# kaleo996/F5E-TTS

Measured on AMD Instinct MI355X. Metric: mel_frames_per_sec, higher is better.
Workload: dtype bf16; 1 GPU; C2: F5TTS_v1_Base random-init, batch 1 per GPU, N_ref=188 N=469 frames, euler NFE=32, CFG=2.0 (cond+uncond batched), sway=-1.0, hipGraph ODE loop, HIP log-mel front-end + Vocos decode on GPU; parallelism=replica x1 (utterance sharding, no collective on the data path)

## Files before the change

f5e-tts_amd/csrc/gemm_bf16.hip:

```cpp
#include <cstdlib>
#include <type_traits>

#include "f5e_common.h"
#include "gemm_bf16_args.h"

namespace {

using namespace f5e_gemm;

template <int N>
__device__ __forceinline__ void wait_vm_lgkm0() {
  asm volatile("s_waitcnt vmcnt(%0) lgkmcnt(0)" ::"n"(N) : "memory");
}

template <int LPT, int EXTRA>
__device__ __forceinline__ void wait_stages(int nst) {
  constexpr auto C = [](int v) constexpr { return v > 63 ? 63 : v; };
  switch (nst) {
    case 0: wait_vm_lgkm0<C(EXTRA)>(); break;
    case 1: wait_vm_lgkm0<C(LPT + EXTRA)>(); break;
    case 2: wait_vm_lgkm0<C(2 * LPT + EXTRA)>(); break;
    case 3: wait_vm_lgkm0<C(3 * LPT + EXTRA)>(); break;
    case 4: wait_vm_lgkm0<C(4 * LPT + EXTRA)>(); break;
    case 5: wait_vm_lgkm0<C(5 * LPT + EXTRA)>(); break;
    default: wait_vm_lgkm0<C(6 * LPT + EXTRA)>(); break;
  }
}

template <int BM, int BN, int EPI, int NSTAGE, int DBG = 0, int WGM = 2, int WGN = 2, int FUSE = 0, int NLOAD = 0, int DSTEP = 1, int DBUF = 1>
__global__ __launch_bounds__(64 * (WGM * WGN + NLOAD)) void gemm_bf16_kernel(GemmArgs a) {
  constexpr int BK = 64;
  constexpr int CPR = BK / 8;
  constexpr int ROWB = BK * 2;
  auto swz = [](int row) { return (row >> 1) & 7; };
  constexpr int NCW = WGM * WGN;
  constexpr int NC = 64 * NCW;
  constexpr int NT = NLOAD ? 64 * NLOAD : NC;
  constexpr int A_BYTES = BM * BK * 2;
  constexpr int W_BYTES = BN * BK * 2;
  constexpr int STAGE = A_BYTES + W_BYTES;
  constexpr int WM = BM / WGM, WN = BN / WGN;
  constexpr int TM = WM / 16, TN = WN / 16;
  extern __shared__ __attribute__((aligned(16))) char smem[];

  const int lane = threadIdx.x & 63;
  const int wave = __builtin_amdgcn_readfirstlane(threadIdx.x >> 6);
  const int tid = (int)threadIdx.x;
  const bool is_loader = NLOAD > 0 && wave >= NCW;
  const int stid = NLOAD ? tid - NC : tid;
  const int swave = NLOAD ? wave - NCW : wave;
  unsigned long long* trc = nullptr;
  if constexpr (DBG >= 3) {
    trc = a.trace + (size_t)blockIdx.x * 48;
    if (tid == 0) { trc[0] = __builtin_amdgcn_s_memrealtime(); trc[1] = __builtin_amdgcn_s_memtime(); }
  }

  if (FUSE == 1)
    asm volatile("" ::"s"(a.ln_stats), "s"(a.ln_c), "s"(a.ln_d), "s"(a.ln_parts), "s"(a.cd_stride), "s"(a.cd_rows),
                 "s"(a.cd_eval_stride), "s"(a.eval_ptr));
  if (EPI == EPI_GATE_RES)
    asm volatile("" ::"s"(a.resid), "s"(a.gate), "s"(a.seq_len), "s"(a.eval_ptr), "s"(a.ldr), "s"(a.gate_stride),
                 "s"(a.gate_rows), "s"(a.eval_stride), "s"(a.bias));
  if (FUSE == 2) asm volatile("" ::"s"(a.next_scale), "s"(a.xs_out), "s"(a.stats_out), "s"(a.ld_xs), "s"(a.row_mean));
  if (EPI == EPI_QKV_ROPE) asm volatile("" ::"s"(a.q), "s"(a.k), "s"(a.vt), "s"(a.cos_sin), "s"(a.n_pad), "s"(a.heads), "s"(a.rope_heads));

  if ((int)blockIdx.x >= a.n_main) {
    if (NLOAD > 0 && a.pf_per_wg) f5e_prefetch_run_packed(a.pf, (int)blockIdx.x - a.n_main, tid, 64 * (NCW + NLOAD), a.pf_per_wg, smem);
    else if (tid < 256) f5e_prefetch_run(a.pf, (int)blockIdx.x - a.n_main, tid, smem);
    return;
  }
  int bid = blockIdx.x;
  {
    const int nblk = a.n_main;
    const int q8 = nblk >> 3, r8 = nblk & 7;
    const int xcd = bid & 7, idx = bid >> 3;
    bid = (xcd < r8 ? xcd * (q8 + 1) : r8 * (q8 + 1) + (xcd - r8) * q8) + idx;
  }
  int tile_m, tile_n;
  if (a.m_major > 0) {
    tile_m = div_magic(bid, a.tiles_n, a.tile_magic);
    tile_n = bid - tile_m * a.tiles_n;
  } else {
    const int sh = -a.m_major, per = a.tiles_m << sh;
    const int g = div_magic(bid, per, a.tile_magic);
    const int r = bid - g * per;
    tile_m = r >> sh;
    tile_n = (g << sh) + (r & ((1 << sh) - 1));
  }
  const int m0 = tile_m * BM, n0 = tile_n * BN;

  constexpr int A_IT = BM * CPR / NT;
  constexpr int W_IT = BN * CPR / NT;
  static_assert(A_IT >= 1 && W_IT >= 1 && A_IT * NT == BM * CPR && W_IT * NT == BN * CPR, "tile / thread-count mismatch");
  unsigned a_off[A_IT], w_off[W_IT];
#pragma unroll
  for (int j = 0; j < A_IT; ++j) {
    const int i = (stid & (NT - 1)) + NT * j;
    const int row = i / CPR, c = (i % CPR) ^ swz(row);
    a_off[j] = (unsigned)(min(m0 + row, a.M - 1) - m0) * (unsigned)(a.lda * 2) + (unsigned)c * 16u;
  }
#pragma unroll
  for (int j = 0; j < W_IT; ++j) {
    const int i = (stid & (NT - 1)) + NT * j;
    const int row = i / CPR, c = (i % CPR) ^ swz(row);
    w_off[j] = (unsigned)(min(n0 + row, a.N - 1) - n0) * (unsigned)(a.ldw * 2) + (unsigned)c * 16u;
  }
  const char* const a_base = (const char*)(a.A + (size_t)m0 * a.lda);
  const char* const w_base = (const char*)(a.W + (size_t)n0 * a.ldw);
  const int KT = a.K / BK;
  char* const ring = smem;
  auto stage = [&](int buf, int kt) {
    char* base = ring + buf * STAGE;
    const char* ak = a_base + (size_t)kt * (BK * 2);
    const char* wk = w_base + (size_t)kt * (BK * 2);
#pragma unroll
    for (int j = 0; j < A_IT; ++j) glds16_s(ak, a_off[j], base + (swave * 64 + NT * j) * 16);
#pragma unroll
    for (int j = 0; j < W_IT; ++j) glds16_s(wk, w_off[j], base + A_BYTES + (swave * 64 + NT * j) * 16);
  };

  const int wm0 = (wave / WGN) * WM, wn0 = (wave % WGN) * WN;
  const int fr = lane & 15, fq = lane >> 4;

  f32x4 acc[TN][TM];
#pragma unroll
  for (int i = 0; i < TN; ++i)
#pragma unroll
    for (int j = 0; j < TM; ++j) acc[i][j] = f32x4{0.f, 0.f, 0.f, 0.f};

  constexpr int LPT = A_IT + W_IT;
  static_assert(NSTAGE >= 2 && NSTAGE <= 8 && (DSTEP > 1 || (NSTAGE - 2) * LPT <= 63), "vmcnt is a 6-bit counter");
  static_assert((NT & (NT - 1)) == 0, "staging thread count must be a power of two");
  static_assert(DSTEP == 1 || (NLOAD > 0 && DSTEP == 2 && NSTAGE >= 3 * DSTEP), "DSTEP: role split, ring of >= 3 steps");
  constexpr int NPRO = NSTAGE - DSTEP;
  static_assert((NSTAGE - 2 * DSTEP) * LPT <= 63, "vmcnt is a 6-bit counter");
  if (NLOAD == 0 || is_loader) {
#pragma unroll
    for (int s = 0; s < NPRO; ++s)
      if (s < KT) stage(s, s);
  }
  if constexpr (NLOAD > 0) {
    if (is_loader) {
      int nbuf_l = NPRO % NSTAGE;
      if constexpr (DBG >= 3) { if (stid == 0) trc[47] = __builtin_amdgcn_s_memtime(); }
      for (int kt = 0; kt < KT; kt += DSTEP) {
        const int rem = KT - DSTEP - kt;
        wait_stages<LPT, 0>(rem < NSTAGE - 2 * DSTEP ? (rem < 0 ? 0 : rem) : NSTAGE - 2 * DSTEP);
        __builtin_amdgcn_s_barrier();
#pragma unroll
        for (int d = 0; d < DSTEP; ++d) {
          if (kt + NPRO + d < KT) stage(nbuf_l, kt + NPRO + d);
          nbuf_l = (nbuf_l + 1 == NSTAGE) ? 0 : nbuf_l + 1;
        }
      }
      if (FUSE == 1) __syncthreads();
      if (FUSE == 2) __builtin_amdgcn_s_barrier();
      return;
    }
  }
  asm volatile("" ::: "memory");
  if constexpr (DBG >= 3) { if (tid == 0) trc[46] = __builtin_amdgcn_s_memtime(); }
  constexpr bool PREF = (TM * TN <= 4);
  static_assert(FUSE != 2 || (PREF && WM == 32 && WN == 32 && BN == 64 && (BM == 64 || (BM == 128 && NLOAD > 0))),
                "fused AdaLN producer: 64 (or, role split, 128) x 64 tiles of 32 x 32 wave sub-tiles");
  static_assert(FUSE != 1 || (WN == 32 && (BN == 64 || NLOAD > 0) && ((BM == 64 && WM == 32) || (BM == 128 && WM == 64 && NLOAD > 0))),
                "fused AdaLN consumer: 64-row tiles of 32 x 32 wave sub-tiles, or (role split) 128-row tiles of 64 x 32 ones");
  static_assert(DBUF == 1 || (NLOAD > 0 && DSTEP == 1), "single fragment set: role split, one tile per hand-over");
  constexpr int NSTATT = BM * 4;
  static_assert(FUSE != 1 || NSTATT <= NC, "fused consumer: 4 statistics threads per row");
  static_assert(FUSE != 2 || EPI == EPI_GATE_RES, "the AdaLN producer is the gate+residual epilogue");
  constexpr int NPC = NLOAD ? 0 : (FUSE == 1 ? 2 * TN + 4 : (FUSE == 2 ? 3 * TM * TN : ((PREF && EPI == EPI_GATE_RES) ? 2 * TM * TN : 0)));
  static_assert((NSTAGE - 2) * LPT + NPC <= 63, "vmcnt is a 6-bit counter");
  constexpr bool COLG = NLOAD > 0;
  f32x4 pf_bias[PREF ? TN : 1], pf_gate[PREF ? TN : 1][PREF ? (COLG ? 1 : TM) : 1], pf_x[PREF ? TN : 1][PREF ? TM : 1];
  f32x4 pf_c[FUSE == 1 ? TN : 1], pf_d[FUSE == 1 ? TN : 1];
  f32x4 pf_ns[FUSE == 2 ? TN : 1][FUSE == 2 ? (COLG ? 1 : TM) : 1];
  f32x2 pf_st[FUSE == 1 ? 4 : 1];
  bool pf_live[PREF ? TM : 1];
  int pf_len[PREF ? TM : 1];
  float pf_rm[FUSE == 2 ? TM : 1];
  auto ldv4 = [](const float* ptr) -> f32x4 { return *(const f32x4*)ptr; };
  auto fetch_epilogue_operands = [&]() {
    if (PREF) {
      if (EPI == EPI_GATE_RES) {
        const size_t eoff = a.eval_ptr ? (size_t)load_uniform_i32(a.eval_ptr) * a.eval_stride : 0;
#pragma unroll
        for (int j = 0; j < TM; ++j) {
          const int m = m0 + wm0 + j * 16 + fr, mc = min(m, a.M - 1);
          const int seq = div_magic(mc, a.rows_per_seq, a.rps_magic);
#pragma unroll
          for (int i = 0; i < TN; ++i) {
            const int nc = min(n0 + wn0 + i * 16 + fq * 4, a.N - 4);
            const size_t goff = eoff + ((COLG || a.gate_rows == 1) ? 0 : (size_t)(seq % a.gate_rows) * a.gate_stride) + nc;
            if (!COLG || j == 0) pf_gate[i][COLG ? 0 : j] = ldv4(a.gate + goff);
            pf_x[i][j] = ldv4(a.resid + (size_t)mc * a.ldr + nc);
            if (FUSE == 2 && (!COLG || j == 0)) pf_ns[i][COLG ? 0 : j] = ldv4(a.next_scale + goff);
          }
        }
      }
    }
    if (FUSE == 1) {
      const size_t eoff = a.eval_ptr ? (size_t)load_uniform_i32(a.eval_ptr) * a.cd_eval_stride : 0;
      const float* cbase = a.ln_c + eoff;
      const float* dbase = a.ln_d + eoff;
#pragma unroll
      for (int i = 0; i < TN; ++i) {
        const unsigned nc = (unsigned)min(n0 + wn0 + i * 16 + fq * 4, a.N - 4);
        pf_c[i] = ldv4(cbase + nc);
        pf_d[i] = ldv4(dbase + nc);
      }
      const int pp = a.ln_parts >> 2;
      const float* sbase = a.ln_stats + (size_t)m0 * a.ln_parts * 2;
      const unsigned rel_max = (unsigned)((a.M - m0) * a.ln_parts - 1);
#pragma unroll
      for (int u = 0; u < 4; ++u) {
        const unsigned rel = min((unsigned)((tid & (NSTATT - 1)) * pp + min(u, pp - 1)), rel_max);
        if (NC == NSTATT || tid < NSTATT) pf_st[u] = *(const f32x2*)(sbase + rel * 2u);
      }
    }
    if (PREF) {
#pragma unroll
      for (int i = 0; i < TN; ++i) {
        const int n = n0 + wn0 + i * 16 + fq * 4;
        pf_bias[i] = (a.bias && n < a.N) ? *(const f32x4*)(a.bias + n) : f32x4{0.f, 0.f, 0.f, 0.f};
      }
      if (EPI == EPI_GATE_RES) {
#pragma unroll
        for (int j = 0; j < TM; ++j) {
          const int mc = min(m0 + wm0 + j * 16 + fr, a.M - 1);
          pf_len[j] = a.seq_len ? a.seq_len[div_magic(mc, a.rows_per_seq, a.rps_magic)] : a.rows_per_seq;
          if (FUSE == 2) pf_rm[j] = a.row_mean[mc];
        }
      }
    }
  };
  if (NLOAD == 0) fetch_epilogue_operands();

  int buf = 0, nbuf = NSTAGE - 1;
  if constexpr (DBG >= 3) { if (tid == 0) trc[2] = __builtin_amdgcn_s_memtime(); }
  if constexpr (NLOAD > 0) {
    bf16x8 xs2[DBUF + 1][BK / 32][TM], ws2[DBUF + 1][BK / 32][TN];
    auto reads = [&](auto pc, int b) {
      constexpr int P = decltype(pc)::value;
      const char* As = ring + b * STAGE;
      const char* Ws = As + A_BYTES;
#pragma unroll
      for (int kk = 0; kk < BK / 32; ++kk) {
        const int c = kk * 4 + fq;
#pragma unroll
        for (int j = 0; j < TM; ++j) {
          const int row = wm0 + j * 16 + fr;
          xs2[P][kk][j] = *(const bf16x8*)(As + row * ROWB + ((c ^ swz(row)) << 4));
        }
#pragma unroll
        for (int i = 0; i < TN; ++i) {
          const int row = wn0 + i * 16 + fr;
          ws2[P][kk][i] = *(const bf16x8*)(Ws + row * ROWB + ((c ^ swz(row)) << 4));
        }
      }
    };
    auto mfmas = [&](auto pc) {
      constexpr int P = decltype(pc)::value;
#pragma unroll
      for (int kk = 0; kk < BK / 32; ++kk)
#pragma unroll
        for (int i = 0; i < TN; ++i)
#pragma unroll
          for (int j = 0; j < TM; ++j)
            acc[i][j] = __builtin_amdgcn_mfma_f32_16x16x32_bf16(ws2[P][kk][i], xs2[P][kk][j], acc[i][j], 0, 0, 0);
    };
    auto body = [&](auto pc, int kt) {
      constexpr int P = decltype(pc)::value;
      if (DSTEP == 1 || P == 0) __builtin_amdgcn_s_barrier();
      if constexpr (DBG >= 3) { if (tid == 0 && kt < 36) trc[4 + kt] = __builtin_amdgcn_s_memtime(); }
      reads(pc, buf);
      if (kt > 0) mfmas(std::integral_constant<int, 1 - P>{});
      if (DSTEP == 1 || P == 1) asm volatile("s_waitcnt lgkmcnt(0)" ::: "memory");
      buf = (buf + 1 == NSTAGE) ? 0 : buf + 1;
    };
    if constexpr (DBUF == 0) {
      auto reads_half = [&](int kk, int b) {
        if constexpr (DBG == 5) return;
        const char* As = ring + b * STAGE;
        const char* Ws = As + A_BYTES;
        const int c = kk * 4 + fq;
#pragma unroll
        for (int j = 0; j < TM; ++j) {
          const int row = wm0 + j * 16 + fr;
          xs2[0][kk][j] = *(const bf16x8*)(As + row * ROWB + ((c ^ swz(row)) << 4));
        }
#pragma unroll
        for (int i = 0; i < TN; ++i) {
          const int row = wn0 + i * 16 + fr;
          ws2[0][kk][i] = *(const bf16x8*)(Ws + row * ROWB + ((c ^ swz(row)) << 4));
        }
      };
      auto mfmas_half = [&](int kk) {
        if constexpr (DBG == 4 || DBG == 5) return;
#pragma unroll
        for (int i = 0; i < TN; ++i)
#pragma unroll
          for (int j = 0; j < TM; ++j)
            acc[i][j] = __builtin_amdgcn_mfma_f32_16x16x32_bf16(ws2[0][kk][i], xs2[0][kk][j], acc[i][j], 0, 0, 0);
      };
      static_assert(BK == 64, "half-tile pipelining: two 32-k halves per K-tile");
      for (int kt = 0; kt < KT; ++kt) {
        __builtin_amdgcn_s_barrier();
        if constexpr (DBG >= 3) { if (tid == 0 && kt < 36) trc[4 + kt] = __builtin_amdgcn_s_memtime(); }
        reads_half(0, buf);
        if (kt > 0) mfmas_half(1);
        if (kt == 0) fetch_epilogue_operands();
        asm volatile("s_waitcnt lgkmcnt(0)" ::: "memory");
        reads_half(1, buf);
        mfmas_half(0);
        asm volatile("s_waitcnt lgkmcnt(0)" ::: "memory");
        buf = (buf + 1 == NSTAGE) ? 0 : buf + 1;
      }
      mfmas_half(1);
    } else {
      for (int kt = 0; kt < KT; kt += 2) {
        body(std::integral_constant<int, 0>{}, kt);
        if (kt == 0) fetch_epilogue_operands();
        if (kt + 1 < KT) body(std::integral_constant<int, 1>{}, kt + 1);
      }
      if ((KT - 1) & 1) mfmas(std::integral_constant<int, 1>{});
      else mfmas(std::integral_constant<int, 0>{});
    }
  } else
  for (int kt = 0; kt < KT; ++kt) {
    const int rem = KT - 1 - kt;
    const int nst = rem < NSTAGE - 2 ? rem : NSTAGE - 2;
    if (NPC > 0 && kt <= NSTAGE - 2) wait_stages<LPT, NPC>(nst);
    else wait_stages<LPT, 0>(nst);
    __builtin_amdgcn_s_barrier();
    if constexpr (DBG >= 3) { if (tid == 0 && kt < 36) trc[4 + kt] = __builtin_amdgcn_s_memtime(); }
    const bool more = kt + NSTAGE - 1 < KT;
    const char* As = ring + buf * STAGE;
    const char* Ws = As + A_BYTES;
    bf16x8 xf[BK / 32][TM], wf[BK / 32][TN];
#pragma unroll
    for (int kk = 0; kk < BK / 32; ++kk) {
      const int c = kk * 4 + fq;
#pragma unroll
      for (int j = 0; j < TM; ++j) {
        const int row = wm0 + j * 16 + fr;
        xf[kk][j] = *(const bf16x8*)(As + row * ROWB + ((c ^ swz(row)) << 4));
      }
#pragma unroll
      for (int i = 0; i < TN; ++i) {
        const int row = wn0 + i * 16 + fr;
        wf[kk][i] = *(const bf16x8*)(Ws + row * ROWB + ((c ^ swz(row)) << 4));
      }
    }
    if (more) stage(nbuf, kt + NSTAGE - 1);
#pragma unroll
    for (int kk = 0; kk < BK / 32; ++kk)
#pragma unroll
      for (int i = 0; i < TN; ++i)
#pragma unroll
        for (int j = 0; j < TM; ++j)
          acc[i][j] = __builtin_amdgcn_mfma_f32_16x16x32_bf16(wf[kk][i], xf[kk][j], acc[i][j], 0, 0, 0);
    buf = (buf + 1 == NSTAGE) ? 0 : buf + 1;
    nbuf = (nbuf + 1 == NSTAGE) ? 0 : nbuf + 1;
  }

  if constexpr (DBG >= 3) { if (tid == 0) trc[3] = __builtin_amdgcn_s_memtime(); }
  float* fuse_lds = (float*)(smem + NSTAGE * STAGE);
  if (FUSE == 1) {
    const int sq = tid & 3, pp = a.ln_parts >> 2;
    float sm = 0.f;
#pragma unroll
    for (int u = 0; u < 4; ++u)
      if (u < pp) sm += pf_st[u][0];
    sm = add_xor2(add_xor1(sm));
    const float mean = sm / (float)a.ln_parts;
    const float cols = (float)(a.K / a.ln_parts);
    float m2 = 0.f;
#pragma unroll
    for (int u = 0; u < 4; ++u)
      if (u < pp) {
        const float dm = pf_st[u][0] - mean;
        m2 += pf_st[u][1] + cols * dm * dm;
      }
    m2 = add_xor2(add_xor1(m2));
    if (sq == 0 && (NC == NSTATT || tid < NSTATT)) {
      fuse_lds[(tid >> 2) * 2] = mean;
      fuse_lds[(tid >> 2) * 2 + 1] = rsqrtf(m2 / (float)a.K + a.ln_eps);
      if (tile_n == 0 && m0 + (tid >> 2) < a.M) a.row_mean[m0 + (tid >> 2)] += mean;
    }
    __syncthreads();
    if constexpr (DBG >= 3) { if (tid == 0) trc[42] = __builtin_amdgcn_s_memtime(); }
  }
  f32x4 xn[FUSE == 2 ? TN : 1][FUSE == 2 ? TM : 1];
  if (PREF && EPI == EPI_GATE_RES) {
#pragma unroll
    for (int j = 0; j < TM; ++j) {
      const int m = m0 + wm0 + j * 16 + fr;
      pf_live[j] = (m < a.M) && (m - div_magic(m, a.rows_per_seq, a.rps_magic) * a.rows_per_seq < pf_len[j]);
    }
  }

  int qkv_which = 0, qkv_head = 0, qkv_d0 = 0;
  bf16* qkv_base = nullptr;
  size_t qkv_seq_stride = 0;
  if (EPI == EPI_QKV_ROPE) {
    static_assert(EPI != EPI_QKV_ROPE || WN <= 64, "a wave's columns must stay inside one 64-wide head");
    const int inner = a.heads * 64, hb = n0 + wn0;
    qkv_which = hb / inner;
    qkv_head = (hb - qkv_which * inner) >> 6;
    qkv_d0 = hb & 63;
    qkv_seq_stride = (size_t)a.heads * a.n_pad * 64;
    qkv_base = (qkv_which == 0 ? a.q : (qkv_which == 1 ? a.k : a.vt)) + (size_t)qkv_head * a.n_pad * 64;
  }

#pragma unroll
  for (int j = 0; j < TM; ++j) {
    const int m = m0 + wm0 + j * 16 + fr;
    if (FUSE == 2) {
#pragma unroll
      for (int i = 0; i < TN; ++i) xn[i][j] = pf_x[i][j];
    }
    if (m >= a.M) continue;
    float ln_mean = 0.f, ln_rstd = 1.f;
    if (FUSE == 1) {
      ln_mean = fuse_lds[(wm0 + j * 16 + fr) * 2];
      ln_rstd = fuse_lds[(wm0 + j * 16 + fr) * 2 + 1];
    }
    int seq = 0, pos = m;
    if (EPI == EPI_GATE_RES || EPI == EPI_QKV_ROPE) {
      seq = div_magic(m, a.rows_per_seq, a.rps_magic);
      pos = m - seq * a.rows_per_seq;
    }
    float qk_rn = 1.0f;
    const float* qk_w = nullptr;
    if constexpr (EPI == EPI_QKV_ROPE && WN == 64) {
      const int which_w = (n0 + wn0) / (a.heads * 64);
      if (a.qn_w && which_w < 2) {
        float ss = 0.f;
#pragma unroll
        for (int i = 0; i < TN; ++i) {
          f32x4 t = acc[i][j];
          if (a.bias) t += *(const f32x4*)(a.bias + n0 + wn0 + i * 16 + fq * 4);
          ss += (t[0] * t[0] + t[1] * t[1]) + (t[2] * t[2] + t[3] * t[3]);
        }
        ss = add_xor32(add_xor16(ss));
        qk_rn = rsqrtf(ss * (1.0f / 64.0f) + a.qk_eps);
        qk_w = which_w == 0 ? a.qn_w : a.kn_w;
      }
    }
#pragma unroll
    for (int i = 0; i < TN; ++i) {
      const int n = n0 + wn0 + i * 16 + fq * 4;
      if (n >= a.N) continue;
      f32x4 v = acc[i][j];
      if (FUSE == 1) {
        v = ln_rstd * (v - ln_mean * pf_c[i]) + pf_d[i];
      } else if (PREF) {
        v += pf_bias[i];
      } else if (a.bias) {
        const f32x4 b = *(const f32x4*)(a.bias + n);
        v += b;
      }
      if (EPI == EPI_BF16) {
        *(bf16x4*)((bf16*)a.out + (size_t)m * a.ldo + n) = f2bf4(v[0], v[1], v[2], v[3]);
      } else if (EPI == EPI_BF16_GELU) {
        *(bf16x4*)((bf16*)a.out + (size_t)m * a.ldo + n) =
            f2bf4(gelu_tanh_f(v[0]), gelu_tanh_f(v[1]), gelu_tanh_f(v[2]), gelu_tanh_f(v[3]));
      } else if (EPI == EPI_F32) {
        *(f32x4*)((float*)a.out + (size_t)m * a.ldo + n) = v;
      } else if (EPI == EPI_GATE_RES && PREF) {
        if (pf_live[j]) {
          const f32x4 x_new = pf_x[i][j] + pf_gate[i][COLG ? 0 : j] * v;
          *(f32x4*)(a.resid + (size_t)m * a.ldr + n) = x_new;
          if (FUSE == 2) xn[i][j] = x_new;
        }
        if (FUSE == 2) {
          const f32x4 y = (xn[i][j] - pf_rm[j]) * (1.0f + pf_ns[i][COLG ? 0 : j]);
          *(bf16x4*)(a.xs_out + (size_t)m * a.ld_xs + n) = f2bf4(y[0], y[1], y[2], y[3]);
        }
      } else if (EPI == EPI_GATE_RES) {
        const bool live = (a.seq_len == nullptr) || (pos < a.seq_len[seq]);
        if (live) {
          const size_t eoff = a.eval_ptr ? (size_t)load_uniform_i32(a.eval_ptr) * a.eval_stride : 0;
          const f32x4 g = *(const f32x4*)(a.gate + eoff + (size_t)(seq % a.gate_rows) * a.gate_stride + n);
          float* xp = a.resid + (size_t)m * a.ldr + n;
          f32x4 x = *(const f32x4*)xp;
          x += g * v;
          *(f32x4*)xp = x;
        }
      } else if (EPI == EPI_QKV_ROPE) {
        const int d = qkv_d0 + i * 16 + fq * 4;
        if (qk_w) v = v * qk_rn * *(const f32x4*)(qk_w + d);
        if (qkv_which < 2) {
          if (qkv_head < a.rope_heads) {
            const f32x4 cs = *(const f32x4*)(a.cos_sin + (size_t)pos * 64 + d);
            const float x0 = v[0], x1 = v[1], x2 = v[2], x3 = v[3];
            v[0] = x0 * cs[0] - x1 * cs[1];
            v[1] = x1 * cs[0] + x0 * cs[1];
            v[2] = x2 * cs[2] - x3 * cs[3];
            v[3] = x3 * cs[2] + x2 * cs[3];
          }
          if (qkv_which == 0) v *= a.q_scale;
          const int off = (pos >> 5) * 2048 + (pos & 31) * 16 + (d >> 4) * 512 + ((d >> 3) & 1) * 8 + (d & 7);
          *(bf16x4*)(qkv_base + (size_t)seq * qkv_seq_stride + off) = f2bf4(v[0], v[1], v[2], v[3]);
        } else {
          const int k16 = pos & 15;
          const int off = (pos >> 4) * 1024 + (d >> 5) * 512 + (d & 31) * 16 + ((k16 >> 2) & 1) * 8 + (((k16 >> 3) << 2) | (k16 & 3));
          bf16* dst = qkv_base + (size_t)seq * qkv_seq_stride + off;
          dst[0] = (bf16)v[0];
          dst[16] = (bf16)v[1];
          dst[32] = (bf16)v[2];
          dst[48] = (bf16)v[3];
        }
      }
    }
  }
  if constexpr (DBG >= 3) { if (tid == 0) trc[43] = __builtin_amdgcn_s_memtime(); }
  if (FUSE == 2) {
#pragma unroll
    for (int j = 0; j < TM; ++j) {
      float sm = 0.f;
#pragma unroll
      for (int i = 0; i < TN; ++i) sm += (xn[i][j][0] + xn[i][j][1]) + (xn[i][j][2] + xn[i][j][3]);
      sm = add_xor32(add_xor16(sm));
      const float mw = sm * (1.0f / (float)WN);
      float q2 = 0.f;
#pragma unroll
      for (int i = 0; i < TN; ++i) {
        const f32x4 dv = xn[i][j] - mw;
        q2 += (dv[0] * dv[0] + dv[1] * dv[1]) + (dv[2] * dv[2] + dv[3] * dv[3]);
      }
      q2 = add_xor32(add_xor16(q2));
      if (fq == 0) {
        float* slot = fuse_lds + ((wm0 + j * 16 + fr) * WGN + (wave % WGN)) * 2;
        slot[0] = mw - pf_rm[j];
        slot[1] = q2;
      }
    }
    if constexpr (DBG >= 3) { if (tid == 0) trc[44] = __builtin_amdgcn_s_memtime(); }
    asm volatile("s_waitcnt lgkmcnt(0)" ::: "memory");
    __builtin_amdgcn_s_barrier();
    if constexpr (DBG >= 3) { if (tid == 0) trc[45] = __builtin_amdgcn_s_memtime(); }
    if (tid < BM && m0 + tid < a.M) {
      const float ma = fuse_lds[tid * 4], qa = fuse_lds[tid * 4 + 1], mb = fuse_lds[tid * 4 + 2], qb = fuse_lds[tid * 4 + 3];
      const float dm = ma - mb;
      float* dst = a.stats_out + ((size_t)(m0 + tid) * a.tiles_n + tile_n) * 2;
      dst[0] = 0.5f * (ma + mb);
      dst[1] = (qa + qb) + (0.25f * (float)BN) * dm * dm;
    }
  }
  if constexpr (DBG >= 3) {
    asm volatile("s_waitcnt vmcnt(0)" ::: "memory");
    if (tid == 0) { trc[40] = __builtin_amdgcn_s_memtime(); trc[41] = __builtin_amdgcn_s_memrealtime(); }
  }
}

inline int pick_group_shift(int tiles_m, int tiles_n, int bm, int bn) {
  struct Memo { int tm, tn, bm, bn, s; };
  static thread_local Memo memo[4] = {};
  static thread_local int next = 0;
  for (const Memo& e : memo)
    if (e.tm == tiles_m && e.tn == tiles_n && e.bm == bm && e.bn == bn) return e.s;
#ifdef F5E_TOOLS
  if (const char* f = getenv("F5E_GEMM_GROUP_SHIFT")) {
    const int s = atoi(f);
    if (s >= 0 && s <= 4 && tiles_n % (1 << s) == 0) return s;
  }
#endif
  const int n = tiles_m * tiles_n, q8 = n >> 3, r8 = n & 7;
  long best = -1;
  int best_s = 0;
  for (int s = 0; s <= 4 && (tiles_n % (1 << s)) == 0 && (1 << s) <= tiles_n; ++s) {
    long cost = 0;
    int id = 0;
    for (int x = 0; x < 8; ++x) {
      const int cnt = q8 + (x < r8 ? 1 : 0);
      unsigned long long seen_m[4] = {}, seen_n[4] = {};
      for (int i = 0; i < cnt; ++i, ++id) {
        const int per = tiles_m << s, g = id / per, r = id - g * per;
        const int tm = r >> s, tn = (g << s) + (r & ((1 << s) - 1));
        seen_m[(tm >> 6) & 3] |= 1ull << (tm & 63);
        seen_n[(tn >> 6) & 3] |= 1ull << (tn & 63);
      }
      for (int w = 0; w < 4; ++w) cost += (long)__builtin_popcountll(seen_m[w]) * bm + (long)__builtin_popcountll(seen_n[w]) * bn;
    }
    if (best < 0 || cost < best) { best = cost; best_s = s; }
  }
  memo[next] = Memo{tiles_m, tiles_n, bm, bn, best_s};
  next = (next + 1) & 3;
  return best_s;
}

inline bool pack_prefetch_on() {
#ifdef F5E_TOOLS
  if (const char* f = getenv("F5E_PF_PACK")) return atoi(f) != 0;
#endif
  return true;
}

template <int BM, int BN, int EPI, int NSTAGE, int WGM = 2, int WGN = 2, int DBG = 0, int FUSE = 0, int NLOAD = 0, int DSTEP = 1, int DBUF = 1>
int launch(GemmArgs& a, hipStream_t st) {
  constexpr int BK = 64;
  a.tiles_m = (a.M + BM - 1) / BM;
  a.tiles_n = (a.N + BN - 1) / BN;
  if (a.M > a.N) {
    a.m_major = 1;
    a.tile_magic = div_magic_of(a.tiles_n);
  } else {
    const int sh = (a.tiles_m <= 256 && a.tiles_n <= 256) ? pick_group_shift(a.tiles_m, a.tiles_n, BM, BN) : 0;
    a.m_major = -sh;
    a.tile_magic = div_magic_of(a.tiles_m << sh);
  }
  a.rps_magic = div_magic_of(a.rows_per_seq);
  a.n_main = a.tiles_m * a.tiles_n;
  int pf_wgs = ((WGM * WGN == 4 || NLOAD > 0) && a.n_main <= 3 * 256) ? f5e_prefetch_wgs(&a.pf) : 0;
  a.pf_per_wg = 0;
  constexpr int lds = NSTAGE * (BM + BN) * BK * 2 + (FUSE ? BM * 16 : 0);
  if (NLOAD > 0 && 2 * lds > 160 * 1024 && pf_wgs > 0 && pack_prefetch_on()) {
    const int idle = f5e_cu_count() - a.n_main;
    if (idle <= 0) {
      pf_wgs = 0;
    } else if (pf_wgs > idle) {
      constexpr unsigned gran = 64u * (WGM * WGN + NLOAD) * 16u;
      const unsigned long long total = (unsigned long long)pf_wgs * F5E_PF_BYTES_PER_WG;
      a.pf_per_wg = (unsigned)(((total + idle - 1) / idle + gran - 1) / gran * gran);
      pf_wgs = (int)((total + a.pf_per_wg - 1) / a.pf_per_wg);
    }
  }
  const int grid = a.n_main + pf_wgs;
  if (grid == a.n_main) a.pf = F5ePrefetch{};
  static_assert(lds <= 160 * 1024, "LDS budget");
  static F5eDeviceOnce lds_once;
  if (lds > 65536) F5E_OPT_IN_LDS(lds_once, (gemm_bf16_kernel<BM, BN, EPI, NSTAGE, DBG, WGM, WGN, FUSE, NLOAD, DSTEP, DBUF>), lds);
  hipLaunchKernelGGL((gemm_bf16_kernel<BM, BN, EPI, NSTAGE, DBG, WGM, WGN, FUSE, NLOAD, DSTEP, DBUF>), dim3(grid), dim3(64 * (WGM * WGN + NLOAD)), lds, st, a);
  F5E_LAUNCH_CHECK("gemm_bf16");
  return F5E_OK;
}

inline bool role_split_on() {
#ifdef F5E_TOOLS
  if (const char* f = getenv("F5E_GEMM_ROLE")) return atoi(f) != 0;
#endif
  return true;
}
inline int role_var() {
#ifdef F5E_TOOLS
  if (const char* f = getenv("F5E_GEMM_VAR")) return atoi(f);
#endif
  return -1;
}

inline bool big_tiles_on() {
#ifdef F5E_TOOLS
  if (const char* f = getenv("F5E_GEMM_BIG")) return atoi(f) != 0;
#endif
  return true;
}

template <int EPI>
int dispatch(GemmArgs& a, hipStream_t st, int tile_hint) {
  auto blocks = [&](int bm, int bn) { return ((a.M + bm - 1) / bm) * ((a.N + bn - 1) / bn); };
  int sel = tile_hint;
  F5E_REQUIRE(sel == 0 || sel == 1 || sel == 2 || sel == 3 || sel == 9, "gemm_bf16: unknown tile_hint %d (0, 1, 2, 3 or 9)", tile_hint);
  if (a.ln_stats || a.stats_out) {
    F5E_REQUIRE(!(a.ln_stats && a.stats_out), "gemm_bf16: a launch is an AdaLN consumer or a producer, not both");
    F5E_REQUIRE(!(EPI == EPI_QKV_ROPE && a.qn_w), "gemm_bf16: fused AdaLN and qk_norm need different tiles");
    if constexpr (EPI == EPI_GATE_RES) {
      F5E_REQUIRE(a.stats_out && !a.ln_stats, "gemm_bf16: the gate+residual epilogue is the AdaLN producer");
      if (role_split_on() && a.gate_rows == 1 && blocks(64, 64) <= 256) {
        if (a.K % 128 == 0 && role_var() != 0) return launch<64, 64, EPI, 6, 2, 2, 0, 2, 4, 2>(a, st);
        return launch<64, 64, EPI, 4, 2, 2, 0, 2, 4, 1>(a, st);
      }
      if (role_split_on() && a.gate_rows == 1 && big_tiles_on() && blocks(128, 64) <= 256) {
        if (a.K % 128 == 0) return launch<128, 64, EPI, 6, 4, 2, 0, 2, 4, 2>(a, st);
        return launch<128, 64, EPI, 4, 4, 2, 0, 2, 4, 1>(a, st);
      }
      if (a.K >= 2048 && blocks(64, 64) <= 256) return launch<64, 64, EPI, 4, 2, 2, 0, 2>(a, st);
      return launch<64, 64, EPI, 3, 2, 2, 0, 2>(a, st);
    } else {
      F5E_REQUIRE(a.ln_stats && !a.stats_out, "gemm_bf16: this epilogue can only consume AdaLN statistics");
      if (role_split_on()) {
        int wide = 3;
#ifdef F5E_TOOLS
        if (const char* f = getenv("F5E_GEMM_WIDE")) wide = atoi(f);
#endif
        if constexpr (EPI == EPI_QKV_ROPE) {
          if ((wide & 1) && a.N % 192 == 0 && blocks(64, 192) <= 256) {
            return launch<64, 192, EPI, 4, 2, 6, 0, 1, 4, 1>(a, st);
          }
          if (big_tiles_on() && a.N % 192 == 0 && blocks(128, 192) <= 256) return launch<128, 192, EPI, 3, 2, 6, 0, 1, 4, 1, 0>(a, st);
        } else {
          if ((wide & 2) && a.N % 128 == 0 && blocks(64, 128) <= 256) {
#ifdef F5E_TOOLS
            if (role_var() == 0) return launch<64, 128, EPI, 3, 2, 4, 0, 1, 4, 1>(a, st);
#endif
            if (a.K % 128 == 0) return launch<64, 128, EPI, 6, 2, 4, 0, 1, 4, 2>(a, st);
          }
          if (big_tiles_on() && a.N % 128 == 0 && blocks(128, 128) <= 256) return launch<128, 128, EPI, 4, 2, 4, 0, 1, 4, 1, 0>(a, st);
        }
      }
      return launch<64, 64, EPI, 3, 2, 2, 0, 1>(a, st);
    }
  }
  if (sel == 9 || (sel == 0 && uses_pp(a.M, a.K))) return launch_pp(EPI, a, st);
  if (EPI == EPI_QKV_ROPE && a.qn_w) sel = 1;
  if (sel == 0) {
    if (blocks(128, 128) >= 320) sel = 1;
    else if (blocks(128, 64) >= 512) sel = 2;
    else sel = 3;
  }
  if (sel == 1) return launch<128, 128, EPI, 2, 4, 2>(a, st);
  if (sel == 2) return launch<128, 64, EPI, 3>(a, st);
  if constexpr (EPI == EPI_GATE_RES) {
    if (role_split_on() && a.gate_rows == 1 && blocks(64, 64) <= 256) return launch<64, 64, EPI, 4, 2, 2, 0, 0, 4>(a, st);
  }
  if (a.K >= 2048 && blocks(64, 64) <= 256) return launch<64, 64, EPI, 4>(a, st);
  return launch<64, 64, EPI, 3>(a, st);
}

int check_common(const GemmArgs& a) {
  F5E_REQUIRE(a.M > 0 && a.N > 0 && a.K > 0, "gemm_bf16: empty problem M=%d N=%d K=%d", a.M, a.N, a.K);
  F5E_REQUIRE(a.K % 64 == 0, "gemm_bf16: K=%d must be a multiple of 64", a.K);
  F5E_REQUIRE(a.N % 4 == 0, "gemm_bf16: N=%d must be a multiple of 4", a.N);
  F5E_REQUIRE(a.lda % 8 == 0 && a.ldw % 8 == 0, "gemm_bf16: lda/ldw must be multiples of 8 elements");
  F5E_REQUIRE(a.A && a.W, "gemm_bf16: null operand");
  return F5E_OK;
}

int set_consumer(GemmArgs& a, const f5e_ln_fuse* ln, const float* bias) {
  if (!ln || !ln->stats) return F5E_OK;
  F5E_REQUIRE(bias == nullptr, "gemm_bf16: with fused AdaLN the bias is part of the d table");
  F5E_REQUIRE(ln->c && ln->d && ln->parts > 0 && ln->parts <= 16 && ln->parts % 4 == 0 && ln->cd_rows == 1 && a.K % ln->parts == 0 && ln->cd_rows > 0 &&
                  ln->cd_stride % 4 == 0 && ln->cd_eval_stride % 4 == 0 && ln->rows_per_seq > 0,
              "gemm_bf16: bad fused-AdaLN consumer arguments (parts=%d: a multiple of 4 up to 16; one table row per evaluation)",
              ln->parts);
  a.ln_stats = ln->stats; a.ln_parts = ln->parts; a.ln_c = ln->c; a.ln_d = ln->d; a.cd_stride = ln->cd_stride;
  a.cd_rows = ln->cd_rows; a.cd_eval_stride = ln->cd_eval_stride; a.ln_eps = ln->eps;
  a.eval_ptr = ln->eval_ptr;
  F5E_REQUIRE(ln->row_mean, "gemm_bf16: the fused-AdaLN consumer needs f5e_ln_fuse.row_mean (the rows' centring offsets)");
  a.row_mean = ln->row_mean;
  if (a.rows_per_seq <= 0) a.rows_per_seq = ln->rows_per_seq;
  return F5E_OK;
}

}

int f5e_gemm_bf16_bias_pf(hipStream_t st, const void* A, int lda, const void* W, int ldw, const float* bias, void* out,
                          int ldo, int M, int N, int K, int act, int out_f32, int tile_hint, const f5e_ln_fuse* ln,
                          const F5ePrefetch* pf) {
  GemmArgs a{};
  if (pf) a.pf = *pf;
  a.A = (const bf16*)A; a.lda = lda; a.W = (const bf16*)W; a.ldw = ldw; a.bias = bias;
  a.M = M; a.N = N; a.K = K; a.out = out; a.ldo = ldo;
  if (int e = check_common(a)) return e;
  if (int e = set_consumer(a, ln, bias)) return e;
  F5E_REQUIRE(out && ldo % 4 == 0, "gemm_bf16_bias: bad output");
  if (out_f32) {
    F5E_REQUIRE(act == F5E_ACT_NONE, "gemm_bf16_bias: f32 output supports no activation");
    return dispatch<EPI_F32>(a, st, tile_hint);
  }
  if (act == F5E_ACT_GELU_TANH) return dispatch<EPI_BF16_GELU>(a, st, tile_hint);
  F5E_REQUIRE(act == F5E_ACT_NONE, "gemm_bf16_bias: unsupported activation %d", act);
  return dispatch<EPI_BF16>(a, st, tile_hint);
}

int f5e_gemm_bf16_gate_residual_pf(hipStream_t st, const void* A, int lda, const void* W, int ldw, const float* bias,
                                   float* resid, int ldr, const float* gate, int gate_stride, int gate_rows,
                                   const int* eval_ptr, int eval_stride, int rows_per_seq, const int* seq_len, int M,
                                   int N, int K, int tile_hint, const f5e_ln_fuse* ln, const F5ePrefetch* pf) {
  GemmArgs a{};
  if (pf) a.pf = *pf;
  a.A = (const bf16*)A; a.lda = lda; a.W = (const bf16*)W; a.ldw = ldw; a.bias = bias;
  a.M = M; a.N = N; a.K = K;
  a.resid = resid; a.ldr = ldr; a.gate = gate; a.gate_stride = gate_stride; a.gate_rows = gate_rows;
  a.rows_per_seq = rows_per_seq; a.seq_len = seq_len; a.eval_ptr = eval_ptr; a.eval_stride = eval_stride;
  if (int e = check_common(a)) return e;
  F5E_REQUIRE(resid && gate && ldr % 4 == 0 && gate_stride % 4 == 0 && gate_rows > 0 && rows_per_seq > 0,
              "gemm_bf16_gate_residual: bad residual/gate arguments");
  if (ln && ln->stats_out) {
    F5E_REQUIRE(ln->xs_out && ln->next_scale && ln->row_mean && ln->ld_xs % 4 == 0 && N % 64 == 0,
                "gemm_bf16_gate_residual: AdaLN producer needs xs_out, next_scale, row_mean and N %% 64 == 0");
    a.xs_out = (bf16*)ln->xs_out; a.ld_xs = ln->ld_xs; a.next_scale = ln->next_scale; a.stats_out = ln->stats_out;
    a.row_mean = ln->row_mean;
  }
  return dispatch<EPI_GATE_RES>(a, st, tile_hint);
}

int f5e_gemm_bf16_qkv_rope_pf(hipStream_t st, const void* A, int lda, const void* W, int ldw, const float* bias, void* q,
                              void* k, void* vt, int n_pad, int heads, int rope_heads, const float* cos_sin,
                              const float* q_norm_w, const float* k_norm_w, int rows_per_seq, int M, int K, int tile_hint,
                              const f5e_ln_fuse* ln, const F5ePrefetch* pf) {
  GemmArgs a{};
  if (pf) a.pf = *pf;
  a.A = (const bf16*)A; a.lda = lda; a.W = (const bf16*)W; a.ldw = ldw; a.bias = bias;
  a.M = M; a.N = 3 * heads * 64; a.K = K;
  a.q = (bf16*)q; a.k = (bf16*)k; a.vt = (bf16*)vt; a.n_pad = n_pad; a.heads = heads; a.rope_heads = rope_heads;
  a.cos_sin = cos_sin; a.rows_per_seq = rows_per_seq;
  a.qn_w = q_norm_w; a.kn_w = k_norm_w; a.qk_eps = 1e-6f;
  a.q_scale = 0.125f * 1.4426950408889634f;
// ... 56 lines not shown
```

Before: 13010 mel-frames/s.

## Stage fused-AdaLN epilogue operands into LDS via loader-wave DMA

In the role-split fused AdaLN GEMMs, the loader waves now issue global_load_lds DMAs at kernel start. These bring the epilogue operands (residual tile, gate/next_scale/bias rows, row means, seq lengths, LN statistics, c/d tables, RoPE cos/sin) into an extra LDS region. Compute waves then read these operands from LDS instead of issuing their own global loads during the main loop, which is meant to take VMEM traffic and register pressure off the MFMA waves. The block-count thresholds also change from a hard-coded 256 to the queried CU count, which can alter tile selection on MI355X. The cost is extra LDS per block, more complex vmcnt accounting in the loader loop, and new barrier handling when KT <= NPRO.

```diff
diff --git a/f5e-tts_amd/csrc/gemm_bf16.hip b/f5e-tts_amd/csrc/gemm_bf16.hip
--- a/f5e-tts_amd/csrc/gemm_bf16.hip
+++ b/f5e-tts_amd/csrc/gemm_bf16.hip
@@ -27,7 +27,25 @@
   }
 }
 
-template <int BM, int BN, int EPI, int NSTAGE, int DBG = 0, int WGM = 2, int WGN = 2, int FUSE = 0, int NLOAD = 0, int DSTEP = 1, int DBUF = 1>
+template <int BM, int BN, int EPI, int FUSE>
+struct StagedMap {
+  static constexpr bool QKV = FUSE == 1 && EPI == EPI_QKV_ROPE;
+  static constexpr int X = 0, X_B = FUSE == 2 ? BM * BN * 4 : 0;
+  static constexpr int ROWS = X + X_B, ROWS_B = FUSE == 2 ? 1024 : 0;
+  static constexpr int RM = ROWS + ROWS_B, RM_B = FUSE == 2 ? 256 : 0;
+  static constexpr int LEN = RM + RM_B, LEN_B = FUSE == 2 ? 256 : 0;
+  static constexpr int ST = LEN + LEN_B, ST_B = FUSE == 1 ? BM * 128 : 0;
+  static constexpr int CD = ST + ST_B, CD_I = FUSE == 1 ? (2 * BN * 4 + 1023) / 1024 : 0, CD_B = CD_I * 1024;
+  static constexpr int ROPE = CD + CD_B, ROPE_B = QKV ? BM * 256 : 0;
+  static constexpr int BYTES = ROPE + ROPE_B;
+};
+
+__device__ __forceinline__ void glds4(const void* g, void* lds) {
+  __builtin_amdgcn_global_load_lds((const __attribute__((address_space(1))) void*)g,
+                                   (__attribute__((address_space(3))) void*)lds, 4, 0, 0);
+}
+
+template <int BM, int BN, int EPI, int NSTAGE, int DBG = 0, int WGM = 2, int WGN = 2, int FUSE = 0, int NLOAD = 0, int DSTEP = 1, int DBUF = 1, int STG = 0>
 __global__ __launch_bounds__(64 * (WGM * WGN + NLOAD)) void gemm_bf16_kernel(GemmArgs a) {
   constexpr int BK = 64;
   constexpr int CPR = BK / 8;
@@ -42,6 +60,11 @@
   constexpr int WM = BM / WGM, WN = BN / WGN;
   constexpr int TM = WM / 16, TN = WN / 16;
   extern __shared__ __attribute__((aligned(16))) char smem[];
+  constexpr bool STAGED = STG != 0;
+  using SM = StagedMap<BM, BN, EPI, FUSE>;
+  static_assert(!STAGED || (NLOAD == 4 && BM == 64 && DBUF == 1 && (FUSE == 1 || (FUSE == 2 && BN == 64))),
+                "staged operands: 4 loader waves, 64-row tiles, fused AdaLN");
+  constexpr int OPS_OFF = NSTAGE * STAGE + (FUSE ? BM * 16 : 0);
 
   const int lane = threadIdx.x & 63;
   const int wave = __builtin_amdgcn_readfirstlane(threadIdx.x >> 6);
@@ -143,15 +166,96 @@
     if (is_loader) {
       int nbuf_l = NPRO % NSTAGE;
       if constexpr (DBG >= 3) { if (stid == 0) trc[47] = __builtin_amdgcn_s_memtime(); }
-      for (int kt = 0; kt < KT; kt += DSTEP) {
-        const int rem = KT - DSTEP - kt;
-        wait_stages<LPT, 0>(rem < NSTAGE - 2 * DSTEP ? (rem < 0 ? 0 : rem) : NSTAGE - 2 * DSTEP);
-        __builtin_amdgcn_s_barrier();
-#pragma unroll
-        for (int d = 0; d < DSTEP; ++d) {
-          if (kt + NPRO + d < KT) stage(nbuf_l, kt + NPRO + d);
-          nbuf_l = (nbuf_l + 1 == NSTAGE) ? 0 : nbuf_l + 1;
-        }
+      auto loader_loop = [&](auto ec) {
+        constexpr int E = decltype(ec)::value;
+        static_assert((NSTAGE - 2 * DSTEP) * LPT + E <= 63, "vmcnt is a 6-bit counter");
+        if constexpr (STAGED) asm volatile("; f5e_staged_loop %0" ::"n"(E) : "memory");
+        for (int kt = 0; kt < KT; kt += DSTEP) {
+          const int rem = KT - DSTEP - kt;
+          const int nst = rem < NSTAGE - 2 * DSTEP ? (rem < 0 ? 0 : rem) : NSTAGE - 2 * DSTEP;
+          if (E > 0 && kt + DSTEP <= NPRO) wait_stages<LPT, E>(nst);
+          else wait_stages<LPT, 0>(nst);
+          __builtin_amdgcn_s_barrier();
+#pragma unroll
+          for (int d = 0; d < DSTEP; ++d) {
+            if (kt + NPRO + d < KT) stage(nbuf_l, kt + NPRO + d);
+            nbuf_l = (nbuf_l + 1 == NSTAGE) ? 0 : nbuf_l + 1;
+          }
+        }
+      };
+      if constexpr (STAGED) {
+        asm volatile("; f5e_staged_begin" ::: "memory");
+        char* const ops = smem + OPS_OFF;
+        using std::integral_constant;
+        if constexpr (FUSE == 2) {
+          constexpr int EB = BM * BN * 4 / 4096;
+#pragma unroll
+          for (int j = 0; j < EB; ++j) {
+            const int t = swave + 4 * j, i = t * 64 + lane, row = i >> 4, c = (i & 15) ^ (row & 15);
+            glds16(a.resid + (size_t)min(m0 + row, a.M - 1) * a.ldr + min(n0 + c * 4, a.N - 4), ops + SM::X + t * 1024);
+          }
+          const int mc = min(m0 + lane, a.M - 1);
+          if (swave == 0) {
+            const size_t eoff = a.eval_ptr ? (size_t)load_uniform_i32(a.eval_ptr) * a.eval_stride : 0;
+            const int part = lane >> 4, nc = min(n0 + (lane & 15) * 4, a.N - 4);
+            const float* src = part == 1 ? a.next_scale + eoff + nc : ((part == 2 && a.bias) ? a.bias + nc : a.gate + eoff + nc);
+            glds16(src, ops + SM::ROWS);
+            loader_loop(integral_constant<int, EB + 1>{});
+          } else if (swave == 1) {
+            glds4(a.row_mean + mc, ops + SM::RM);
+            loader_loop(integral_constant<int, EB + 1>{});
+          } else if (swave == 2) {
+            glds4(a.seq_len ? (const void*)(a.seq_len + div_magic(mc, a.rows_per_seq, a.rps_magic)) : (const void*)(a.row_mean + mc), ops + SM::LEN);
+            loader_loop(integral_constant<int, EB + 1>{});
+          } else {
+            loader_loop(integral_constant<int, EB>{});
+          }
+        } else {
+          constexpr int EB = SM::ST_B / 4096, ER = SM::ROPE_B / 4096;
+          const int vch = (min(BM, a.M - m0) * a.ln_parts) >> 1;
+          const char* sbase = (const char*)(a.ln_stats + (size_t)m0 * a.ln_parts * 2);
+#pragma unroll
+          for (int j = 0; j < EB; ++j) {
+            const int t = swave + 4 * j, i = t * 64 + lane;
+            glds16(sbase + (size_t)min(i, vch - 1) * 16, ops + SM::ST + t * 1024);
+          }
+          static_assert(SM::CD_I <= 4, "c | d rows: at most one DMA per loader wave");
+          auto stage_cd = [&]() {
+            const size_t eoff = a.eval_ptr ? (size_t)load_uniform_i32(a.eval_ptr) * a.cd_eval_stride : 0;
+            const int gch = min(swave * 64 + lane, 2 * (BN / 4) - 1);
+            const bool isd = gch >= BN / 4;
+            const int nc = min(n0 + (gch - (isd ? BN / 4 : 0)) * 4, a.N - 4);
+            glds16((isd ? a.ln_d : a.ln_c) + eoff + nc, ops + SM::CD + swave * 1024);
+          };
+          if (SM::QKV && n0 < 2 * a.heads * 64 && a.rope_heads > 0) {
+#pragma unroll
+            for (int j = 0; j < ER; ++j) {
+              const int t = swave + 4 * j, i = t * 64 + lane, row = i >> 4, c = (i & 15) ^ (row & 15);
+              const int mc = min(m0 + row, a.M - 1);
+              const int pos = mc - div_magic(mc, a.rows_per_seq, a.rps_magic) * a.rows_per_seq;
+              glds16(a.cos_sin + (size_t)pos * 64 + c * 4, ops + SM::ROPE + t * 1024);
+            }
+            if (swave < SM::CD_I) {
+              stage_cd();
+              loader_loop(integral_constant<int, EB + ER + 1>{});
+            } else {
+              loader_loop(integral_constant<int, EB + ER>{});
+            }
+          } else {
+            if (swave < SM::CD_I) {
+              stage_cd();
+              loader_loop(integral_constant<int, EB + 1>{});
+            } else {
+              loader_loop(integral_constant<int, EB>{});
+            }
+          }
+        }
+        if (KT <= NPRO) {
+          asm volatile("s_waitcnt vmcnt(0)" ::: "memory");
+          __builtin_amdgcn_s_barrier();
+        }
+      } else {
+        loader_loop(std::integral_constant<int, 0>{});
       }
       if (FUSE == 1) __syncthreads();
       if (FUSE == 2) __builtin_amdgcn_s_barrier();
@@ -181,6 +285,7 @@
   float pf_rm[FUSE == 2 ? TM : 1];
   auto ldv4 = [](const float* ptr) -> f32x4 { return *(const f32x4*)ptr; };
   auto fetch_epilogue_operands = [&]() {
+    if constexpr (STAGED) return;
     if (PREF) {
       if (EPI == EPI_GATE_RES) {
         const size_t eoff = a.eval_ptr ? (size_t)load_uniform_i32(a.eval_ptr) * a.eval_stride : 0;
@@ -309,7 +414,7 @@
         if constexpr (DBG >= 3) { if (tid == 0 && kt < 36) trc[4 + kt] = __builtin_amdgcn_s_memtime(); }
         reads_half(0, buf);
         if (kt > 0) mfmas_half(1);
-        if (kt == 0) fetch_epilogue_operands();
+        if (!STAGED && kt == 0) fetch_epilogue_operands();
         asm volatile("s_waitcnt lgkmcnt(0)" ::: "memory");
         reads_half(1, buf);
         mfmas_half(0);
@@ -320,7 +425,7 @@
     } else {
       for (int kt = 0; kt < KT; kt += 2) {
         body(std::integral_constant<int, 0>{}, kt);
-        if (kt == 0) fetch_epilogue_operands();
+        if (!STAGED && kt == 0) fetch_epilogue_operands();
         if (kt + 1 < KT) body(std::integral_constant<int, 1>{}, kt + 1);
       }
       if ((KT - 1) & 1) mfmas(std::integral_constant<int, 1>{});
@@ -365,6 +470,45 @@
   }
 
   if constexpr (DBG >= 3) { if (tid == 0) trc[3] = __builtin_amdgcn_s_memtime(); }
+  if constexpr (STAGED) {
+    if (KT <= NPRO) __builtin_amdgcn_s_barrier();
+    asm volatile("" ::: "memory");
+    const char* const ops = smem + OPS_OFF;
+    if constexpr (FUSE == 2) {
+#pragma unroll
+      for (int j = 0; j < TM; ++j) {
+        const int row = wm0 + j * 16 + fr;
+#pragma unroll
+        for (int i = 0; i < TN; ++i) {
+          const int c = (wn0 >> 2) + i * 4 + fq;
+          pf_x[i][j] = *(const f32x4*)(ops + SM::X + row * (BN * 4) + ((c ^ (row & 15)) << 4));
+        }
+        pf_len[j] = a.seq_len ? *(const int*)(ops + SM::LEN + row * 4) : a.rows_per_seq;
+        pf_rm[j] = *(const float*)(ops + SM::RM + row * 4);
+      }
+#pragma unroll
+      for (int i = 0; i < TN; ++i) {
+        const int cb = (wn0 + i * 16 + fq * 4) * 4;
+        pf_gate[i][0] = *(const f32x4*)(ops + SM::ROWS + cb);
+        pf_ns[i][0] = *(const f32x4*)(ops + SM::ROWS + 256 + cb);
+        pf_bias[i] = a.bias ? *(const f32x4*)(ops + SM::ROWS + 512 + cb) : f32x4{0.f, 0.f, 0.f, 0.f};
+      }
+    } else {
+#pragma unroll
+      for (int i = 0; i < TN; ++i) {
+        const int cb = (wn0 + i * 16 + fq * 4) * 4;
+        pf_c[i] = *(const f32x4*)(ops + SM::CD + cb);
+        pf_d[i] = *(const f32x4*)(ops + SM::CD + BN * 4 + cb);
+      }
+      const int pp = a.ln_parts >> 2;
+      const unsigned rel_max = (unsigned)((a.M - m0) * a.ln_parts - 1);
+#pragma unroll
+      for (int u = 0; u < 4; ++u) {
+        const unsigned rel = min((unsigned)((tid & (NSTATT - 1)) * pp + min(u, pp - 1)), rel_max);
+        if (NC == NSTATT || tid < NSTATT) pf_st[u] = *(const f32x2*)(ops + SM::ST + rel * 8u);
+      }
+    }
+  }
   float* fuse_lds = (float*)(smem + NSTAGE * STAGE);
   if (FUSE == 1) {
     const int sq = tid & 3, pp = a.ln_parts >> 2;
@@ -493,7 +637,13 @@
         if (qk_w) v = v * qk_rn * *(const f32x4*)(qk_w + d);
         if (qkv_which < 2) {
           if (qkv_head < a.rope_heads) {
-            const f32x4 cs = *(const f32x4*)(a.cos_sin + (size_t)pos * 64 + d);
+            f32x4 cs;
+            if constexpr (STAGED) {
+              const int row = wm0 + j * 16 + fr;
+              cs = *(const f32x4*)(smem + OPS_OFF + SM::ROPE + row * 256 + (((d >> 2) ^ (row & 15)) << 4));
+            } else {
+              cs = *(const f32x4*)(a.cos_sin + (size_t)pos * 64 + d);
+            }
             const float x0 = v[0], x1 = v[1], x2 = v[2], x3 = v[3];
             v[0] = x0 * cs[0] - x1 * cs[1];
             v[1] = x1 * cs[0] + x0 * cs[1];
@@ -598,7 +748,7 @@
   return true;
 }
 
-template <int BM, int BN, int EPI, int NSTAGE, int WGM = 2, int WGN = 2, int DBG = 0, int FUSE = 0, int NLOAD = 0, int DSTEP = 1, int DBUF = 1>
+template <int BM, int BN, int EPI, int NSTAGE, int WGM = 2, int WGN = 2, int DBG = 0, int FUSE = 0, int NLOAD = 0, int DSTEP = 1, int DBUF = 1, int STG = 0>
 int launch(GemmArgs& a, hipStream_t st) {
   constexpr int BK = 64;
   a.tiles_m = (a.M + BM - 1) / BM;
@@ -613,9 +763,9 @@
   }
   a.rps_magic = div_magic_of(a.rows_per_seq);
   a.n_main = a.tiles_m * a.tiles_n;
-  int pf_wgs = ((WGM * WGN == 4 || NLOAD > 0) && a.n_main <= 3 * 256) ? f5e_prefetch_wgs(&a.pf) : 0;
+  int pf_wgs = ((WGM * WGN == 4 || NLOAD > 0) && a.n_main <= 3 * f5e_cu_count()) ? f5e_prefetch_wgs(&a.pf) : 0;
   a.pf_per_wg = 0;
-  constexpr int lds = NSTAGE * (BM + BN) * BK * 2 + (FUSE ? BM * 16 : 0);
+  constexpr int lds = NSTAGE * (BM + BN) * BK * 2 + (FUSE ? BM * 16 : 0) + (STG ? StagedMap<BM, BN, EPI, FUSE>::BYTES : 0);
   if (NLOAD > 0 && 2 * lds > 160 * 1024 && pf_wgs > 0 && pack_prefetch_on()) {
     const int idle = f5e_cu_count() - a.n_main;
     if (idle <= 0) {
@@ -631,8 +781,8 @@
   if (grid == a.n_main) a.pf = F5ePrefetch{};
   static_assert(lds <= 160 * 1024, "LDS budget");
   static F5eDeviceOnce lds_once;
-  if (lds > 65536) F5E_OPT_IN_LDS(lds_once, (gemm_bf16_kernel<BM, BN, EPI, NSTAGE, DBG, WGM, WGN, FUSE, NLOAD, DSTEP, DBUF>), lds);
-  hipLaunchKernelGGL((gemm_bf16_kernel<BM, BN, EPI, NSTAGE, DBG, WGM, WGN, FUSE, NLOAD, DSTEP, DBUF>), dim3(grid), dim3(64 * (WGM * WGN + NLOAD)), lds, st, a);
+  if (lds > 65536) F5E_OPT_IN_LDS(lds_once, (gemm_bf16_kernel<BM, BN, EPI, NSTAGE, DBG, WGM, WGN, FUSE, NLOAD, DSTEP, DBUF, STG>), lds);
+  hipLaunchKernelGGL((gemm_bf16_kernel<BM, BN, EPI, NSTAGE, DBG, WGM, WGN, FUSE, NLOAD, DSTEP, DBUF, STG>), dim3(grid), dim3(64 * (WGM * WGN + NLOAD)), lds, st, a);
   F5E_LAUNCH_CHECK("gemm_bf16");
   return F5E_OK;
 }
@@ -660,6 +810,7 @@
 template <int EPI>
 int dispatch(GemmArgs& a, hipStream_t st, int tile_hint) {
   auto blocks = [&](int bm, int bn) { return ((a.M + bm - 1) / bm) * ((a.N + bn - 1) / bn); };
+  const int cus = f5e_cu_count();
   int sel = tile_hint;
   F5E_REQUIRE(sel == 0 || sel == 1 || sel == 2 || sel == 3 || sel == 9, "gemm_bf16: unknown tile_hint %d (0, 1, 2, 3 or 9)", tile_hint);
   if (a.ln_stats || a.stats_out) {
@@ -667,15 +818,15 @@
     F5E_REQUIRE(!(EPI == EPI_QKV_ROPE && a.qn_w), "gemm_bf16: fused AdaLN and qk_norm need different tiles");
     if constexpr (EPI == EPI_GATE_RES) {
       F5E_REQUIRE(a.stats_out && !a.ln_stats, "gemm_bf16: the gate+residual epilogue is the AdaLN producer");
-      if (role_split_on() && a.gate_rows == 1 && blocks(64, 64) <= 256) {
-        if (a.K % 128 == 0 && role_var() != 0) return launch<64, 64, EPI, 6, 2, 2, 0, 2, 4, 2>(a, st);
-        return launch<64, 64, EPI, 4, 2, 2, 0, 2, 4, 1>(a, st);
-      }
-      if (role_split_on() && a.gate_rows == 1 && big_tiles_on() && blocks(128, 64) <= 256) {
+      if (role_split_on() && a.gate_rows == 1 && blocks(64, 64) <= cus) {
+        if (a.K % 128 == 0 && role_var() != 0) return launch<64, 64, EPI, 6, 2, 2, 0, 2, 4, 2, 1, 1>(a, st);
+        return launch<64, 64, EPI, 4, 2, 2, 0, 2, 4, 1, 1, 1>(a, st);
+      }
+      if (role_split_on() && a.gate_rows == 1 && big_tiles_on() && blocks(128, 64) <= cus) {
         if (a.K % 128 == 0) return launch<128, 64, EPI, 6, 4, 2, 0, 2, 4, 2>(a, st);
         return launch<128, 64, EPI, 4, 4, 2, 0, 2, 4, 1>(a, st);
       }
-      if (a.K >= 2048 && blocks(64, 64) <= 256) return launch<64, 64, EPI, 4, 2, 2, 0, 2>(a, st);
+      if (a.K >= 2048 && blocks(64, 64) <= cus) return launch<64, 64, EPI, 4, 2, 2, 0, 2>(a, st);
       return launch<64, 64, EPI, 3, 2, 2, 0, 2>(a, st);
     } else {
       F5E_REQUIRE(a.ln_stats && !a.stats_out, "gemm_bf16: this epilogue can only consume AdaLN statistics");
@@ -685,18 +836,18 @@
         if (const char* f = getenv("F5E_GEMM_WIDE")) wide = atoi(f);
 #endif
         if constexpr (EPI == EPI_QKV_ROPE) {
-          if ((wide & 1) && a.N % 192 == 0 && blocks(64, 192) <= 256) {
-            return launch<64, 192, EPI, 4, 2, 6, 0, 1, 4, 1>(a, st);
+          if ((wide & 1) && a.N % 192 == 0 && blocks(64, 192) <= cus) {
+            return launch<64, 192, EPI, 4, 2, 6, 0, 1, 4, 1, 1, 1>(a, st);
           }
-          if (big_tiles_on() && a.N % 192 == 0 && blocks(128, 192) <= 256) return launch<128, 192, EPI, 3, 2, 6, 0, 1, 4, 1, 0>(a, st);
+          if (big_tiles_on() && a.N % 192 == 0 && blocks(128, 192) <= cus) return launch<128, 192, EPI, 3, 2, 6, 0, 1, 4, 1, 0>(a, st);
         } else {
-          if ((wide & 2) && a.N % 128 == 0 && blocks(64, 128) <= 256) {
+          if ((wide & 2) && a.N % 128 == 0 && blocks(64, 128) <= cus) {
 #ifdef F5E_TOOLS
             if (role_var() == 0) return launch<64, 128, EPI, 3, 2, 4, 0, 1, 4, 1>(a, st);
 #endif
-            if (a.K % 128 == 0) return launch<64, 128, EPI, 6, 2, 4, 0, 1, 4, 2>(a, st);
+            if (a.K % 128 == 0) return launch<64, 128, EPI, 6, 2, 4, 0, 1, 4, 2, 1, 1>(a, st);
           }
-          if (big_tiles_on() && a.N % 128 == 0 && blocks(128, 128) <= 256) return launch<128, 128, EPI, 4, 2, 4, 0, 1, 4, 1, 0>(a, st);
+          if (big_tiles_on() && a.N % 128 == 0 && blocks(128, 128) <= cus) return launch<128, 128, EPI, 4, 2, 4, 0, 1, 4, 1, 0>(a, st);
         }
       }
       return launch<64, 64, EPI, 3, 2, 2, 0, 1>(a, st);
@@ -712,9 +863,9 @@
   if (sel == 1) return launch<128, 128, EPI, 2, 4, 2>(a, st);
   if (sel == 2) return launch<128, 64, EPI, 3>(a, st);
   if constexpr (EPI == EPI_GATE_RES) {
-    if (role_split_on() && a.gate_rows == 1 && blocks(64, 64) <= 256) return launch<64, 64, EPI, 4, 2, 2, 0, 0, 4>(a, st);
-  }
-  if (a.K >= 2048 && blocks(64, 64) <= 256) return launch<64, 64, EPI, 4>(a, st);
+    if (role_split_on() && a.gate_rows == 1 && blocks(64, 64) <= cus) return launch<64, 64, EPI, 4, 2, 2, 0, 0, 4>(a, st);
+  }
+  if (a.K >= 2048 && blocks(64, 64) <= cus) return launch<64, 64, EPI, 4>(a, st);
   return launch<64, 64, EPI, 3>(a, st);
 }
 
```

After: 13030 mel-frames/s, median of 2. No clear change (+0.1%).
